# leggedrobotics/delora

Measured on AMD Instinct MI355X. Metric: training scan-pairs/sec, KITTI 64x2048 range images, higher is better.
Workload: dtype f32; 1 GPU; KITTI-shaped 64x2048, batch=8 pairs/GPU, raw scans of ~141k points (ragged, raster order), steps rotate over 8 distinct HBM-resident batches, online normals, ResNet pose CNN (11.9M params, identity-pretrained state), Adam; BASELINE configs[1]; global_batch=8, parallelism=dp1, cnn=fp32, cnn_impl=hip trunk: fp32 MFMA, fused Winograd F(2x2,3x3) + direct implicit GEMM, channels_last=False, hip_graph=False, distinct_batches=8, priming_steps=8

## Files before the change

delora_amd/_lib.py:

```python
import ctypes
import os

_HERE = os.path.dirname(os.path.abspath(__file__))
LIB_PATH = os.path.join(_HERE, "csrc", "libdelora_hip.so")
ABI_VERSION = 10


class DeloraHipError(RuntimeError):
    pass


class SensorStruct(ctypes.Structure):
    _fields_ = [("H", ctypes.c_int32), ("W", ctypes.c_int32),
                ("hfov0", ctypes.c_double), ("hfov1", ctypes.c_double),
                ("vfov0", ctypes.c_double), ("vfov1", ctypes.c_double)]


_vp, _i32, _i64, _u32, _f32, _sz = (ctypes.c_void_p, ctypes.c_int32, ctypes.c_int64, ctypes.c_uint32,
                                    ctypes.c_float, ctypes.c_size_t)
_SP = ctypes.POINTER(SensorStruct)

SIGNATURES = {
    "dl_abi_version": (_i32, []),
    "dl_last_error": (ctypes.c_char_p, []),
# ... 44 lines not shown
    "dl_wino_weights_f32": (_i32, [_vp, _vp, _vp, _i32, _i32, _vp]),
    "dl_wino_weights_batch_f32": (_i32, [_vp, _i32, _vp]),
    "dl_wino_conv3x3_workspace_bytes": (_sz, [_i32, _i32, _i32, _i32, _i32]),
    "dl_wino_conv3x3_nhwc_f32": (_i32, [_vp, _vp, _vp, _vp, _vp, _i32, _i32, _i32, _i32, _i32, _i32, _u32, _vp, _vp]),
    "dl_wino_strided_takes": (_i32, [_i32, _i32, _i32, _i32, _i32, _i32, _i32, _i32]),
    "dl_wino_strided_weights_floats": (_sz, [_i32, _i32, _i32, _i32]),
    "dl_wino_strided_weights_f32": (_i32, [_vp, _vp, _vp, _i32, _i32, _i32, _i32, _vp]),
    "dl_wino_strided_conv3x3_nhwc_f32": (_i32, [_vp, _vp, _vp, _i32, _i32, _i32, _i32, _i32, _i32, _i32, _i32, _u32, _vp]),
    "dl_wino_strided_dgrad3x3_nhwc_f32": (_i32, [_vp, _vp, _vp, _vp, _vp, _i32, _i32, _i32, _i32, _i32, _i32, _i32, _i32, _u32, _vp]),
    "dl_wino_wgrad_workspace_bytes": (_sz, [_i32, _i32, _i32, _i32, _i32]),
    "dl_wino_wgrad3x3_nhwc_f32": (_i32, [_vp, _vp, _vp, _vp, _i32, _i32, _i32, _i32, _i32, _vp]),
    "dl_pool3x3s12_nhwc_fwd": (_i32, [_vp, _i32, _i32, _i32, _i32, _vp, _vp, _vp]),
    "dl_pool3x3s12_nhwc_bwd": (_i32, [_vp, _vp, _vp, _i32, _i32, _i32, _i32, _i32, _vp, _vp]),
    "dl_stem_wgrad_workspace_bytes": (_sz, [_i32, _i32, _i32]),
    "dl_stem_wgrad_f32": (_i32, [_vp, _vp, _vp, _vp, _i32, _i32, _i32, _i32, _vp, _vp, _vp]),
    "dl_quat_to_T_fwd": (_i32, [_vp, _vp, _i32, ctypes.c_float, _vp, _vp]),
    "dl_quat_to_T_bwd": (_i32, [_vp, _vp, _i32, ctypes.c_float, _vp, _vp, _vp]),
    "dl_mean_hw_nhwc_f32": (_i32, [_vp, _i32, _i32, _i32, _vp, _vp]),
    "dl_conv_weights_h": (_i32, [_vp, _vp, _vp, _i32, _i32, _i32, _i32, _vp]),
    "dl_conv_weights_batch_h": (_i32, [_vp, _i32, _i32, _vp]),
    "dl_conv2d_nhwc_h": (_i32, [_vp, _vp, _vp, _vp, _vp, _i32, _i32, _i32, _i32, _i32, _i32, _i32, _i32, _i32, _i32, _i32, _u32, _vp]),
    "dl_conv2d_dgrad_strided_nhwc_h": (_i32, [_vp, _vp, _vp, _vp, _vp, _i32, _i32, _i32, _i32, _i32, _i32, _i32, _i32, _i32, _i32, _i32,
                                              _u32, _vp, _vp]),
    "dl_cast_f32_to_h": (_i32, [_vp, _vp, _i64, _i32, _vp]),
    "dl_heads_fwd": (_i32, [_vp, _vp, _i32, _i32, _i32, _i32, _i32, _vp, _vp, _vp, _vp, _vp, _vp, _vp]),
    "dl_heads_bwd_workspace_bytes": (_sz, [_i32, _i32, _i32, _i32]),
    "dl_heads_bwd": (_i32, [_vp, _vp, _i32, _i32, _i32, _i32, _i32, _vp, _vp, _vp, _vp, _vp, _vp, _vp, _vp, _vp, _vp]),
    "dl_heads_fwd_drop": (_i32, [_vp, _vp, _i32, _i32, _i32, _i32, _i32, _vp, _vp, _vp, _vp, _vp, _vp, _vp, _vp]),
    "dl_heads_bwd_drop": (_i32, [_vp, _vp, _i32, _i32, _i32, _i32, _i32, _vp, _vp, _vp, _vp, _vp, _vp, _vp, _vp, _vp, _vp, _vp]),
    "dl_heads_single_fwd": (_i32, [_vp, _vp, _i32, _i32, _i32, _i32, _i32, _i32, _i32, _i32, _vp, _vp, _vp, _vp, _vp, _vp, _vp]),
# ... 142 lines not shown
```

delora_amd/csrc/common.h:

```cpp
#pragma once
#include <hip/hip_runtime.h>
#include <stdint.h>

#include "../../include/delora_hip.h"

#define DL_WAVE 64
#define DL_BLOCK 256

struct SensorK {
  int H, W, HW;
  float hf0f, hspanf, wm1f;
  float vf0f, vspanf, hm1f;
  double hf0, hres, vf0, vres;
  float tol_u, tol_v;
};

static inline SensorK make_sensor(const dl_sensor* s) {
  SensorK k;
  k.H = s->H; k.W = s->W; k.HW = s->H * s->W;
  k.hf0f = (float)s->hfov0; k.hspanf = (float)(s->hfov1 - s->hfov0); k.wm1f = (float)(s->W - 1);
  k.vf0f = (float)s->vfov0; k.vspanf = (float)(s->vfov1 - s->vfov0); k.hm1f = (float)(s->H - 1);
  k.hf0 = s->hfov0; k.hres = (s->hfov1 - s->hfov0) / (double)(s->W - 1);
  k.vf0 = s->vfov0; k.vres = (s->vfov1 - s->vfov0) / (double)(s->H - 1);
  k.tol_u = (float)(3e-6 * fabs((double)k.wm1f / (double)k.hspanf) + 2.4e-7 * (double)s->W);
// ... 39 lines not shown
  p = __builtin_fmaf(p, t, 0.020650655031204224f);
  p = __builtin_fmaf(p, t, -0.05374353006482124f);
  p = __builtin_fmaf(p, t, 0.13331492245197296f);
  p = __builtin_fmaf(p, t, -0.3333328366279602f);
  const float lo = __builtin_fmaf(ax * t, p, ax);
  const float e = __builtin_amdgcn_exp2f(ax * 2.885390081777927f);
  const float hi = __builtin_fmaf(__builtin_amdgcn_rcpf(e + 1.f), -2.f, 1.f);
  return __builtin_copysignf(ax < 0.625f ? lo : hi, x);
}

extern thread_local char g_dl_err[256];
int dl_fail(int code, const char* fmt, ...);
int dl_check_launch(const char* what);
void dl_plan_batch(const int* tiles, const int* chunks, int n, int machines, int partial_cost, int* nslabs);
int dl_fill_words(void* p, uint32_t value, size_t n_words, hipStream_t st);

#include <hip/hip_ext.h>
struct DlProfTag {
  const char* kernel;
  const char* pass;
  int N, H, W, C, K;
  int ks, sh, sw;
  double flop;
  double bytes;
};
bool dl_prof_is_open();
void dl_prof_events(const DlProfTag& tag, hipEvent_t* e0, hipEvent_t* e1);

struct DlPlanSink {
  char* buf;
// ... 26 lines not shown
```

delora_amd/csrc/infer.hip:

```cpp
#include <stdint.h>
#include <stdio.h>
#include <string.h>

#include "common.h"

typedef uint32_t u32x4i __attribute__((ext_vector_type(4)));

__global__ __launch_bounds__(DL_BLOCK) void k_interleave_pair(const uint32_t* __restrict__ prev, size_t prev_ss, const uint32_t* __restrict__ cur,
                                                              size_t cur_ss, uint32_t HW, uint32_t total, u32x4i* __restrict__ x8) {
  const uint32_t i = blockIdx.x * DL_BLOCK + threadIdx.x;
  if (i >= total) return;
  const uint32_t b = i / HW, p = i - b * HW;
  const uint32_t* a = prev + (size_t)b * prev_ss + p;
  const uint32_t* c = cur + (size_t)b * cur_ss + p;
  const u32x4i lo = {a[0], a[HW], a[2 * (size_t)HW], a[3 * (size_t)HW]};
  const u32x4i hi = {c[0], c[HW], c[2 * (size_t)HW], c[3 * (size_t)HW]};
  x8[2 * (size_t)i] = lo;
  x8[2 * (size_t)i + 1] = hi;
}

__global__ void k_single_scan_offsets(int32_t* __restrict__ offs, int32_t n) {
  if (threadIdx.x < 2) offs[threadIdx.x] = threadIdx.x ? n : 0;
}

namespace {

constexpr size_t kAlign = 256;
inline size_t align_up(size_t n) { return (n + kAlign - 1) / kAlign * kAlign; }
inline int ceil_div(int n, int s) { return (n + s - 1) / s; }

int pose_check(const char* who, const dl_pose_net* net, int B, int H, int W) {
  if (!net) return dl_fail(DL_ERR_INVALID_ARGUMENT, "%s: null net", who);
  if (net->act != DL_POSE_ACT_TANH && net->act != DL_POSE_ACT_RELU)
    return dl_fail(DL_ERR_UNSUPPORTED, "%s: act=%d is not served (1 tanh, 2 relu)", who, net->act);
// ... 90 lines not shown
  if (!rc) return DL_OK;
  char inner[160];
  snprintf(inner, sizeof(inner), "%s", g_dl_err);
  if (block >= 0) return dl_fail(rc, "%s: blocks[%d].%s: %s", who, block, what, inner);
  return dl_fail(rc, "%s: %s: %s", who, what, inner);
}

int pose_forward(const char* who, const dl_pose_net* net, const PosePlan& p, const void* prepared, const float* image_prev, int64_t prev_ss,
                 const float* image_cur, int64_t cur_ss, int B, int H, int W, void* workspace, float* translation, float* quaternion, float* T,
                 dl_stream stream) {
  char* const ws = (char*)workspace;
  float* slot[4];
  for (int i = 0; i < 4; ++i) slot[i] = (float*)(ws + p.slot_off[i]);
  void* const split_ws = p.split_bytes ? (void*)(ws + p.split_off) : nullptr;
  const int act = net->act;
  hipStream_t st = (hipStream_t)stream;
  const uint32_t total = (uint32_t)B * H * W;
  hipLaunchKernelGGL(k_interleave_pair, dim3((total + DL_BLOCK - 1) / DL_BLOCK), dim3(DL_BLOCK), 0, st, (const uint32_t*)image_prev, (size_t)prev_ss,
                     (const uint32_t*)image_cur, (size_t)cur_ss, (uint32_t)(H * W), total, (u32x4i*)slot[0]);
  if (int rc = dl_check_launch(who)) return rc;
  if (int rc = at_layer(who, "conv1", -1, dl_conv2d_nhwc_f32(slot[0], net->conv1_w, slot[1], nullptr, nullptr, B, H, W, 8, 64, 3, 1, 2, 0, act, DL_CONV_ACT, stream)))
    return rc;
  if (int rc = at_layer(who, "pooling", -1, dl_pool3x3s12_nhwc_fwd(slot[1], B, H, W / 2, 64, slot[2], (int8_t*)(ws + p.win_off), stream))) return rc;
  const float* u = (const float*)prepared;
  int s = 2, h = H, w = W / 4;
  for (int i = 0; i < net->n_blocks; ++i) {
    const dl_pose_block& b = net->blocks[i];
    const int ho = ceil_div(h, b.stride_h), wo = ceil_div(w, b.stride_w);
    const float* x = slot[s];
    float *y1 = slot[(s + 1) & 3], *sc = slot[(s + 2) & 3], *y2 = slot[(s + 3) & 3];
    int rc;
    if (runs_wino(b.stride_h, b.stride_w)) {
      rc = dl_wino_conv3x3_nhwc_f32(x, u, y1, nullptr, nullptr, B, h, w, b.cin, b.cout, act, DL_CONV_ACT, split_ws, stream);
      u += dl_wino_weights_floats(b.cout, b.cin);
    } else {
      rc = dl_conv2d_nhwc_f32(x, b.w1, y1, nullptr, nullptr, B, h, w, b.cin, b.cout, 3, b.stride_h, b.stride_w, 0, act, DL_CONV_ACT, stream);
    }
    if ((rc = at_layer(who, "w1", i, rc))) return rc;
// ... 118 lines not shown
```

delora_amd/csrc/stem.hip:

```cpp
#include "common.h"

#define ST_TANH 1
#define ST_RELU 2

typedef float f32x4s __attribute__((ext_vector_type(4)));

__global__ __launch_bounds__(DL_BLOCK) void k_pool_nhwc_fwd(const float* __restrict__ a, int H, int Wc, int C4, uint32_t total,
                                                            float* __restrict__ y, int8_t* __restrict__ win) {
  const uint32_t i = blockIdx.x * DL_BLOCK + threadIdx.x;
  if (i >= total) return;
  const int Wp = Wc >> 1;
  const uint32_t pix = i / (uint32_t)C4;
  const int c4 = (int)(i - pix * (uint32_t)C4);
  const uint32_t nr = pix / (uint32_t)Wp;
  const int q = (int)(pix - nr * (uint32_t)Wp);
  const int r = (int)(nr % (uint32_t)H);
  const int first = r > 0 ? 0 : 3;
  f32x4s best = {-INFINITY, -INFINITY, -INFINITY, -INFINITY};
  int k0 = first, k1 = first, k2 = first, k3 = first;
#pragma unroll
  for (int dh = -1; dh <= 1; ++dh) {
    if (r + dh < 0 || r + dh >= H) continue;
    const float* row = a + ((size_t)(nr + dh) * Wc) * (size_t)(4 * C4) + 4 * c4;
#pragma unroll
    for (int dw = -1; dw <= 1; ++dw) {
      int j = 2 * q + dw;
      j = j < 0 ? j + Wc : j;
      const f32x4s v = *reinterpret_cast<const f32x4s*>(row + (size_t)j * (4 * C4));
      const int k = (dh + 1) * 3 + dw + 1;
      if (v.x > best.x || v.x != v.x) { best.x = v.x; k0 = k; }
      if (v.y > best.y || v.y != v.y) { best.y = v.y; k1 = k; }
      if (v.z > best.z || v.z != v.z) { best.z = v.z; k2 = k; }
      if (v.w > best.w || v.w != v.w) { best.w = v.w; k3 = k; }
    }
  }
  *reinterpret_cast<f32x4s*>(y + (size_t)i * 4) = best;
  *reinterpret_cast<uint32_t*>(win + (size_t)i * 4) = (uint32_t)k0 | ((uint32_t)k1 << 8) | ((uint32_t)k2 << 16) | ((uint32_t)k3 << 24);
}

__device__ __forceinline__ f32x4s pool_bwd_value(const float* __restrict__ g, const float* __restrict__ a, const int8_t* __restrict__ win,
                                                 int H, int Wc, int C4, int act, uint32_t nr, int r, int j, int c4) {
  const int Wp = Wc >> 1;
  const int q0 = j >> 1, col0 = 1 + (j & 1);
  const int q1 = (q0 + 1 == Wp) ? 0 : q0 + 1;
  const bool two = (j & 1) != 0;
  uint32_t w4[6];
  f32x4s gv[6];
  uint32_t code[6];
#pragma unroll
  for (int d = -1; d <= 1; ++d) {
    const bool row_ok = r + d >= 0 && r + d < H;
    const size_t rowbase = (size_t)(nr + (row_ok ? d : 0)) * Wp;
#pragma unroll
    for (int t = 0; t < 2; ++t) {
      const int i = (d + 1) * 2 + t;
      const size_t e = ((rowbase + ((t && two) ? q1 : q0)) * (size_t)C4 + c4) * 4;
      w4[i] = *reinterpret_cast<const uint32_t*>(win + e);
      gv[i] = *reinterpret_cast<const f32x4s*>(g + e);
      code[i] = (row_ok && (t == 0 || two)) ? (uint32_t)((1 - d) * 3 + (t ? 0 : col0)) : 0xffu;
    }
  }
  f32x4s acc = {0.f, 0.f, 0.f, 0.f};
#pragma unroll
  for (int i = 0; i < 6; ++i) {
    acc.x += (w4[i] & 0xffu) == code[i] ? gv[i].x : 0.f;
    acc.y += ((w4[i] >> 8) & 0xffu) == code[i] ? gv[i].y : 0.f;
    acc.z += ((w4[i] >> 16) & 0xffu) == code[i] ? gv[i].z : 0.f;
    acc.w += (w4[i] >> 24) == code[i] ? gv[i].w : 0.f;
  }
  const f32x4s av = *reinterpret_cast<const f32x4s*>(a + (((size_t)nr * Wc + j) * C4 + c4) * 4);
  f32x4s out;
  if (act == ST_TANH) {
    out.x = acc.x * (1.f - av.x * av.x); out.y = acc.y * (1.f - av.y * av.y);
    out.z = acc.z * (1.f - av.z * av.z); out.w = acc.w * (1.f - av.w * av.w);
  } else if (act == ST_RELU) {
    out.x = av.x <= 0.f ? 0.f : acc.x; out.y = av.y <= 0.f ? 0.f : acc.y;
    out.z = av.z <= 0.f ? 0.f : acc.z; out.w = av.w <= 0.f ? 0.f : acc.w;
  } else {
    out = acc;
  }
  return out;
}

__global__ __launch_bounds__(DL_BLOCK) void k_pool_nhwc_bwd(const float* __restrict__ g, const float* __restrict__ a,
                                                            const int8_t* __restrict__ win, int H, int Wc, int C4, int act,
                                                            uint32_t total, float* __restrict__ g_conv) {
  const uint32_t i = blockIdx.x * DL_BLOCK + threadIdx.x;
  if (i >= total) return;
  const uint32_t pix = i / (uint32_t)C4;
  const int c4 = (int)(i - pix * (uint32_t)C4);
  const uint32_t nr = pix / (uint32_t)Wc;
  const int j = (int)(pix - nr * (uint32_t)Wc);
  const int r = (int)(nr % (uint32_t)H);
  *reinterpret_cast<f32x4s*>(g_conv + (size_t)i * 4) = pool_bwd_value(g, a, win, H, Wc, C4, act, nr, r, j, c4);
}

#define SG_PX 64
#define SG_XCOLS (2 * SG_PX + 2)
typedef float f32x16s __attribute__((ext_vector_type(16)));

__global__ __launch_bounds__(DL_BLOCK, 2) void k_stem_wgrad(const float* __restrict__ g, const float* __restrict__ a,
                                                            const int8_t* __restrict__ win, const float* __restrict__ x8, int N, int H,
                                                            int Wc, int act, int chunks_per_slab, float* __restrict__ part) {
  constexpr int K = 64, C4 = 16;
  __shared__ __attribute__((aligned(16))) float gc[SG_PX * K];
  __shared__ __attribute__((aligned(16))) float xt[3 * SG_XCOLS * 8];
  const int tid = threadIdx.x, lane = tid & 63, wave = tid >> 6;
  const int li = lane & 31, half = lane >> 5;
  const int W = 2 * Wc;
  const int cpr = (Wc + SG_PX - 1) / SG_PX;
  const int total = N * H * cpr;
  const int ch_begin = blockIdx.x * chunks_per_slab, ch_end = min(ch_begin + chunks_per_slab, total);
  f32x16s acc[2][3];
#pragma unroll
  for (int i = 0; i < 2; ++i)
#pragma unroll
    for (int j = 0; j < 3; ++j)
#pragma unroll
      for (int r = 0; r < 16; ++r) acc[i][j][r] = 0.f;
  int b_off[3];
#pragma unroll
  for (int ns = 0; ns < 3; ++ns) {
    const int j = min(li + 32 * ns, 71), tap = j >> 3, c = j & 7;
    b_off[ns] = ((tap / 3) * SG_XCOLS + (tap % 3)) * 8 + c;
  }
  for (int ch = ch_begin; ch < ch_end; ++ch) {
    const int cb = ch % cpr;
    const uint32_t nr = (uint32_t)(ch / cpr);
    const int h = (int)(nr % (uint32_t)H), wc0 = cb * SG_PX;
    __syncthreads();
#pragma unroll
    for (int it = 0; it < SG_PX * C4 / DL_BLOCK; ++it) {
      const int q = tid + it * DL_BLOCK, pl = q / C4, c4 = q % C4;
      f32x4s v = {0.f, 0.f, 0.f, 0.f};
      if (wc0 + pl < Wc) v = pool_bwd_value(g, a, win, H, Wc, C4, act, nr, h, wc0 + pl, c4);
      *reinterpret_cast<f32x4s*>(gc + pl * K + c4 * 4) = v;
    }
    for (int q = tid; q < 3 * SG_XCOLS * 2; q += DL_BLOCK) {
      const int hp = q & 1, col = (q >> 1) % SG_XCOLS, row = (q >> 1) / SG_XCOLS;
      const int hh = h + row - 1;
      int w = (2 * wc0 - 1 + col) % W;
      w = w < 0 ? w + W : w;
      f32x4s v = {0.f, 0.f, 0.f, 0.f};
      if (hh >= 0 && hh < H) v = *reinterpret_cast<const f32x4s*>(x8 + (((size_t)(nr + row - 1)) * W + w) * 8 + hp * 4);
      *reinterpret_cast<f32x4s*>(xt + (row * SG_XCOLS + col) * 8 + hp * 4) = v;
    }
    __syncthreads();
#pragma unroll
    for (int ks = 0; ks < 8; ++ks) {
      const int pl = wave * 16 + ks * 2 + half;
      const float a0 = gc[pl * K + li], a1 = gc[pl * K + 32 + li];
      float b[3];
#pragma unroll
      for (int ns = 0; ns < 3; ++ns) b[ns] = xt[b_off[ns] + 2 * pl * 8];
#pragma unroll
      for (int ns = 0; ns < 3; ++ns) {
        acc[0][ns] = __builtin_amdgcn_mfma_f32_32x32x2f32(a0, b[ns], acc[0][ns], 0, 0, 0);
        acc[1][ns] = __builtin_amdgcn_mfma_f32_32x32x2f32(a1, b[ns], acc[1][ns], 0, 0, 0);
      }
    }
// ... 108 lines not shown
  if (N <= 0 || H <= 0 || W <= 0 || W % 4) return 0;
  return (size_t)stem_wgrad_slabs(N * H * ((W / 2 + SG_PX - 1) / SG_PX)) * 64 * 72 * sizeof(float);
}

extern "C" int dl_stem_wgrad_f32(const float* g_pooled, const float* a, const int8_t* win, const float* x8, int32_t N, int32_t H,
                                 int32_t W, int32_t act, void* workspace, float* dw, dl_stream stream) {
  if (!g_pooled || !a || !win || !x8 || !workspace || !dw || N <= 0 || H <= 0 || W <= 0 || act < 0 || act > 2)
    return dl_fail(DL_ERR_INVALID_ARGUMENT, "dl_stem_wgrad_f32: bad argument");
  if (W % 4 || (size_t)N * H * W * 32 >= ((size_t)1 << 32))
    return dl_fail(DL_ERR_UNSUPPORTED, "dl_stem_wgrad_f32: N=%d H=%d W=%d not supported (W %% 4, conv1 output below 2^32 elements)", N, H, W);
  const int Wc = W / 2, total = N * H * ((Wc + SG_PX - 1) / SG_PX), nslabs = stem_wgrad_slabs(total);
  const int cps = (total + nslabs - 1) / nslabs, grid = (total + cps - 1) / cps;
  hipStream_t st = (hipStream_t)stream;
  const DlProfTag tag{"k_stem_wgrad", "wgrad", N, H, W, 8, 64, 3, 1, 2, 2.0 * N * H * Wc * 64.0 * 72.0,
                      4.0 * ((double)N * H * Wc * 64 * 1.5 + (double)N * H * W * 8) + (double)N * H * (Wc / 2) * 64};
  DL_LAUNCH(tag, k_stem_wgrad, dim3(grid), dim3(DL_BLOCK), st, g_pooled, a, win, x8, N, H, Wc, act, cps, (float*)workspace);
  hipLaunchKernelGGL(k_stem_wgrad_reduce, dim3(64 * 72 / 64), dim3(DL_BLOCK), 0, st, (const float*)workspace, grid, dw);
  return dl_check_launch("dl_stem_wgrad_f32");
}
```

delora_amd/models/ring_conv.py:

```python
import ctypes
import os

import torch

from .. import _lib

ACT = {"none": 0, "tanh": 1, "relu": 2}
USE_WINOGRAD = True
EPI_ADD, EPI_ACT, EPI_DACT, EPI_ADD_GRID = 1, 2, 4, 8


def _ptr(t):
    return ctypes.c_void_p(t.data_ptr()) if t is not None else ctypes.c_void_p(0)


def _stream():
    return ctypes.c_void_p(torch.cuda.current_stream().cuda_stream)


ALLOC_SKEW = 0
_skew_state = {"i": 0}


def _empty(shape, dtype, device):
# ... 282 lines not shown
    y = torch.empty((N, H, W // 2, C), dtype=torch.float32, device=a.device)
    win = torch.empty((N, H, W // 2, C), dtype=torch.int8, device=a.device)
    _lib.check(lib.dl_pool3x3s12_nhwc_fwd(_ptr(a), N, H, W, C, _ptr(y), _ptr(win), _stream()), "dl_pool3x3s12_nhwc_fwd")
    return y, win


def pool_bwd(g, a, win, act):
    lib = _lib.load()
    N, H, W, C = a.shape
    out = torch.empty_like(a)
    _lib.check(lib.dl_pool3x3s12_nhwc_bwd(_ptr(g), _ptr(a), _ptr(win), N, H, W, C, int(act), _ptr(out), _stream()),
               "dl_pool3x3s12_nhwc_bwd")
    return out


class MeanHW(torch.autograd.Function):

    @staticmethod
    def forward(ctx, x):
        lib = _lib.load()
        x = x.contiguous()
        N, H, W, C = x.shape
        y = torch.empty((N, C), dtype=torch.float32, device=x.device)
        _lib.check(lib.dl_mean_hw_nhwc_f32(_ptr(x), N, H * W, C, _ptr(y), _stream()), "dl_mean_hw_nhwc_f32")
        ctx.shape = (N, H, W, C)
        return y

    @staticmethod
    def backward(ctx, g):
        N, H, W, C = ctx.shape
# ... 79 lines not shown

def stem_supported(x_shape, out_channels):
    N, C, H, W = x_shape
    k_ok = out_channels % 64 == 0 or (C == 8 and out_channels in NARROW_STEM_CHANNELS and N * H * W * 64 < (1 << 31))
    return ((C % 8 == 0 and C % 16 != 0) or C == TOWER_CHANNELS) and k_ok and W % 4 == 0 and W >= 4 and H >= 1


def planar_stem_supported(x_shape, out_channels):
    return stem_supported(x_shape, out_channels) and x_shape[1] % 16 != 0


class RingStem(torch.autograd.Function):

    @staticmethod
    def forward(ctx, x, w1, act, *drop):
        if drop and drop[0] is not None:
            seed, p = drop[0]
            x8 = stem_input_drop(x, seed, p)
            ctx.drop_p = float(p)
        else:
            seed = None
            x8 = x.permute(0, 2, 3, 1).contiguous()
        ctx.n_extra = len(drop)
        conv1 = conv_nhwc if w1.shape[0] % 64 == 0 else narrow_conv
        a = conv1(x8, weight_storage(w1), stride=(1, 2), act=act, epilogue=EPI_ACT if act else 0)
        y, win = pool_fwd(a)
        ctx.save_for_backward(x8, a, win, w1, *([seed] if seed is not None else []))
        ctx.act = act
        return y

    @staticmethod
    def backward(ctx, g):
        x8, a, win, w1, *seed = ctx.saved_tensors
        extra = (None,) * ctx.n_extra
        want_x = ctx.needs_input_grad[0]
        lib = _lib.load()
        N, H, W, _ = x8.shape
        nbytes = 0 if want_x or a.shape[3] != 64 or x8.shape[3] != 8 else lib.dl_stem_wgrad_workspace_bytes(N, H, W)
        if nbytes:
            ws = torch.empty((nbytes // 4,), dtype=torch.float32, device=x8.device)
            dw = torch.empty((64, 8, 3, 3), dtype=torch.float32, device=x8.device)
            _lib.check(lib.dl_stem_wgrad_f32(_ptr(g.contiguous()), _ptr(a), _ptr(win), _ptr(x8), N, H, W, int(ctx.act), _ptr(ws), _ptr(dw),
                                             _stream()), "dl_stem_wgrad_f32")
            return (None, dw, None) + extra
        gc = pool_bwd(g.contiguous(), a, win, ctx.act)
        if not want_x and a.shape[3] % 64:
            dw = narrow_wgrad(x8, gc, 3, stride=(1, 2)).permute(0, 3, 1, 2)
            return (None, dw if tuple(dw.stride()) == tuple(w1.stride()) else dw.contiguous(), None) + extra
        xp = torch.cat((x8[:, :, -1:], x8, x8[:, :, :1]), dim=2).permute(0, 3, 1, 2)
        gx, dw, _ = torch.ops.aten.convolution_backward(gc.permute(0, 3, 1, 2), xp, w1, None, (1, 2), (1, 0), (1, 1), False,
                                                        (0, 0), 1, (want_x, True, False))
        if want_x:
            gxp = gx
            gx = gxp[..., 1:-1].clone()
            gx[..., -1] += gxp[..., 0]
            gx[..., 0] += gxp[..., -1]
            if seed:
                gx = gx * dropout_scale(seed[0], SITE_INPUT, ctx.drop_p, x8.numel()).view(x8.shape).permute(0, 3, 1, 2)
        return ((gx if want_x else None), dw, None) + extra
# ... 603 lines not shown
```

include/delora_hip.h:

```cpp
#ifndef DELORA_HIP_H
#define DELORA_HIP_H

#include <stddef.h>
#include <stdint.h>

#ifdef __cplusplus
extern "C" {
#endif

#define DL_ABI_VERSION 10

typedef void* dl_stream;

typedef enum {
  DL_OK = 0,
  DL_ERR_INVALID_ARGUMENT = -1,
  DL_ERR_LAUNCH = -2,
  DL_ERR_UNSUPPORTED = -3
} dl_status;

typedef struct {
  int32_t H;
  int32_t W;
  double hfov0, hfov1;
// ... 197 lines not shown
int dl_conv2d_wgrad_nhwc_h(const void* x, const void* g, float* dw, void* workspace, int32_t N, int32_t H, int32_t W, int32_t C,
                           int32_t K, int32_t ksize, int32_t stride_h, int32_t stride_w, int32_t dtype, dl_stream stream);

typedef dl_wgrad_layer dl_wgrad_h_layer;
size_t dl_conv2d_wgrad_batch_h_workspace_bytes(const dl_wgrad_h_layer* layers, int32_t n);
int dl_conv2d_wgrad_batch_nhwc_h(const dl_wgrad_h_layer* layers, int32_t n, void* workspace, int32_t dtype, dl_stream stream);

int dl_pool3x3s12_nhwc_fwd(const float* a, int32_t N, int32_t H, int32_t W, int32_t C, float* y, int8_t* win, dl_stream stream);
int dl_pool3x3s12_nhwc_bwd(const float* g, const float* a, const int8_t* win, int32_t N, int32_t H, int32_t W, int32_t C,
                           int32_t act, float* g_conv, dl_stream stream);

size_t dl_stem_wgrad_workspace_bytes(int32_t N, int32_t H, int32_t W);
int dl_stem_wgrad_f32(const float* g_pooled, const float* a, const int8_t* win, const float* x8, int32_t N, int32_t H, int32_t W,
                      int32_t act, void* workspace, float* dw, dl_stream stream);

typedef struct {
  const float *fc_w, *fc_b;
  const float *r1_w, *r1_b;
  const float *r3_w, *r3_b;
  const float *t1_w, *t1_b;
  const float *t3_w, *t3_b;
} dl_heads_params;
int dl_heads_fwd(const float* x, const dl_heads_params* params, int32_t B, int32_t F, int32_t R, int32_t Hd, int32_t act, float* a1,
                 float* a2, float* rot_raw, float* translation, float* rotation, float* norm, dl_stream stream);
size_t dl_heads_bwd_workspace_bytes(int32_t B, int32_t F, int32_t R, int32_t Hd);
int dl_heads_bwd(const float* x, const dl_heads_params* params, int32_t B, int32_t F, int32_t R, int32_t Hd, int32_t act, const float* a1,
                 const float* a2, const float* rot_raw, const float* norm, const float* grad_translation, const float* grad_rotation,
                 const dl_heads_params* grads, float* grad_x, void* workspace, dl_stream stream);

int dl_heads_fwd_drop(const float* x, const dl_heads_params* params, int32_t B, int32_t F, int32_t R, int32_t Hd, int32_t act,
// ... 90 lines not shown
```

Measured before the change: 696.0 scan-pairs/s.

## Fuse stem conv1, activation and max-pool into one kernel reading NCHW input

Adds a fused stem forward kernel that reads the NCHW (or channels-last dropout) input directly, applies the 3x3 stride-(1,2) conv, the activation and the 3x3 pool, and writes only the pooled output plus window indices. The full-resolution conv1 activation and the NHWC permute copy are never materialised. A matching wgrad path rebuilds the activation value from the pooled output and window index instead of reading the saved conv output. The intent is to cut HBM traffic on the largest activation in the network. When the input gradient is needed, backward recomputes conv1, which adds work in that case.

```diff
diff --git a/delora_amd/_lib.py b/delora_amd/_lib.py
--- a/delora_amd/_lib.py
+++ b/delora_amd/_lib.py
@@ -82,6 +82,9 @@
     "dl_pool3x3s12_nhwc_bwd": (_i32, [_vp, _vp, _vp, _i32, _i32, _i32, _i32, _i32, _vp, _vp]),
     "dl_stem_wgrad_workspace_bytes": (_sz, [_i32, _i32, _i32]),
     "dl_stem_wgrad_f32": (_i32, [_vp, _vp, _vp, _vp, _i32, _i32, _i32, _i32, _vp, _vp, _vp]),
+    "dl_stem_fwd_f32": (_i32, [_vp, _i64, _i64, _i64, _i64, _vp, _i32, _i32, _i32, _i32, _vp, _vp, _vp]),
+    "dl_stem_fwd_plan": (_i32, [_i32, _i32, _vp, _vp, _vp, _vp]),
+    "dl_stem_wgrad_y_f32": (_i32, [_vp, _vp, _vp, _vp, _i64, _i64, _i64, _i64, _i32, _i32, _i32, _i32, _vp, _vp, _vp]),
     "dl_quat_to_T_fwd": (_i32, [_vp, _vp, _i32, ctypes.c_float, _vp, _vp]),
     "dl_quat_to_T_bwd": (_i32, [_vp, _vp, _i32, ctypes.c_float, _vp, _vp, _vp]),
     "dl_mean_hw_nhwc_f32": (_i32, [_vp, _i32, _i32, _i32, _vp, _vp]),
diff --git a/delora_amd/csrc/common.h b/delora_amd/csrc/common.h
--- a/delora_amd/csrc/common.h
+++ b/delora_amd/csrc/common.h
@@ -77,6 +77,8 @@
 int dl_check_launch(const char* what);
 void dl_plan_batch(const int* tiles, const int* chunks, int n, int machines, int partial_cost, int* nslabs);
 int dl_fill_words(void* p, uint32_t value, size_t n_words, hipStream_t st);
+int dl_stem_fwd_launch(const char* who, const float* x_lo, int64_t sn_lo, const float* x_hi, int64_t sn_hi, int64_t sc, int64_t sh, int64_t sp,
+                       const float* w, int32_t N, int32_t H, int32_t W, int32_t act, float* y, int8_t* win, dl_stream stream);
 
 #include <hip/hip_ext.h>
 struct DlProfTag {
diff --git a/delora_amd/csrc/infer.hip b/delora_amd/csrc/infer.hip
--- a/delora_amd/csrc/infer.hip
+++ b/delora_amd/csrc/infer.hip
@@ -3,21 +3,6 @@
 #include <string.h>
 
 #include "common.h"
-
-typedef uint32_t u32x4i __attribute__((ext_vector_type(4)));
-
-__global__ __launch_bounds__(DL_BLOCK) void k_interleave_pair(const uint32_t* __restrict__ prev, size_t prev_ss, const uint32_t* __restrict__ cur,
-                                                              size_t cur_ss, uint32_t HW, uint32_t total, u32x4i* __restrict__ x8) {
-  const uint32_t i = blockIdx.x * DL_BLOCK + threadIdx.x;
-  if (i >= total) return;
-  const uint32_t b = i / HW, p = i - b * HW;
-  const uint32_t* a = prev + (size_t)b * prev_ss + p;
-  const uint32_t* c = cur + (size_t)b * cur_ss + p;
-  const u32x4i lo = {a[0], a[HW], a[2 * (size_t)HW], a[3 * (size_t)HW]};
-  const u32x4i hi = {c[0], c[HW], c[2 * (size_t)HW], c[3 * (size_t)HW]};
-  x8[2 * (size_t)i] = lo;
-  x8[2 * (size_t)i + 1] = hi;
-}
 
 __global__ void k_single_scan_offsets(int32_t* __restrict__ offs, int32_t n) {
   if (threadIdx.x < 2) offs[threadIdx.x] = threadIdx.x ? n : 0;
@@ -138,14 +123,9 @@
   for (int i = 0; i < 4; ++i) slot[i] = (float*)(ws + p.slot_off[i]);
   void* const split_ws = p.split_bytes ? (void*)(ws + p.split_off) : nullptr;
   const int act = net->act;
-  hipStream_t st = (hipStream_t)stream;
-  const uint32_t total = (uint32_t)B * H * W;
-  hipLaunchKernelGGL(k_interleave_pair, dim3((total + DL_BLOCK - 1) / DL_BLOCK), dim3(DL_BLOCK), 0, st, (const uint32_t*)image_prev, (size_t)prev_ss,
-                     (const uint32_t*)image_cur, (size_t)cur_ss, (uint32_t)(H * W), total, (u32x4i*)slot[0]);
-  if (int rc = dl_check_launch(who)) return rc;
-  if (int rc = at_layer(who, "conv1", -1, dl_conv2d_nhwc_f32(slot[0], net->conv1_w, slot[1], nullptr, nullptr, B, H, W, 8, 64, 3, 1, 2, 0, act, DL_CONV_ACT, stream)))
+  if (int rc = at_layer(who, "stem", -1, dl_stem_fwd_launch("dl_stem_fwd_f32", image_prev, prev_ss, image_cur, cur_ss, (int64_t)H * W, W, 1, net->conv1_w,
+                                                            B, H, W, act, slot[2], (int8_t*)(ws + p.win_off), stream)))
     return rc;
-  if (int rc = at_layer(who, "pooling", -1, dl_pool3x3s12_nhwc_fwd(slot[1], B, H, W / 2, 64, slot[2], (int8_t*)(ws + p.win_off), stream))) return rc;
   const float* u = (const float*)prepared;
   int s = 2, h = H, w = W / 4;
   for (int i = 0; i < net->n_blocks; ++i) {
diff --git a/delora_amd/csrc/stem.hip b/delora_amd/csrc/stem.hip
--- a/delora_amd/csrc/stem.hip
+++ b/delora_amd/csrc/stem.hip
@@ -38,6 +38,7 @@
   *reinterpret_cast<uint32_t*>(win + (size_t)i * 4) = (uint32_t)k0 | ((uint32_t)k1 << 8) | ((uint32_t)k2 << 16) | ((uint32_t)k3 << 24);
 }
 
+template <bool FROM_Y>
 __device__ __forceinline__ f32x4s pool_bwd_value(const float* __restrict__ g, const float* __restrict__ a, const int8_t* __restrict__ win,
                                                  int H, int Wc, int C4, int act, uint32_t nr, int r, int j, int c4) {
   const int Wp = Wc >> 1;
@@ -47,6 +48,7 @@
   uint32_t w4[6];
   f32x4s gv[6];
   uint32_t code[6];
+  uint32_t eo[6];
 #pragma unroll
   for (int d = -1; d <= 1; ++d) {
     const bool row_ok = r + d >= 0 && r + d < H;
@@ -57,18 +59,35 @@
       const size_t e = ((rowbase + ((t && two) ? q1 : q0)) * (size_t)C4 + c4) * 4;
       w4[i] = *reinterpret_cast<const uint32_t*>(win + e);
       gv[i] = *reinterpret_cast<const f32x4s*>(g + e);
+      eo[i] = (uint32_t)e;
       code[i] = (row_ok && (t == 0 || two)) ? (uint32_t)((1 - d) * 3 + (t ? 0 : col0)) : 0xffu;
     }
   }
   f32x4s acc = {0.f, 0.f, 0.f, 0.f};
+  constexpr uint32_t NONE = 0xffffffffu;
+  uint32_t ex = NONE, ey = NONE, ez = NONE, ew = NONE;
 #pragma unroll
   for (int i = 0; i < 6; ++i) {
-    acc.x += (w4[i] & 0xffu) == code[i] ? gv[i].x : 0.f;
-    acc.y += ((w4[i] >> 8) & 0xffu) == code[i] ? gv[i].y : 0.f;
-    acc.z += ((w4[i] >> 16) & 0xffu) == code[i] ? gv[i].z : 0.f;
-    acc.w += (w4[i] >> 24) == code[i] ? gv[i].w : 0.f;
-  }
-  const f32x4s av = *reinterpret_cast<const f32x4s*>(a + (((size_t)nr * Wc + j) * C4 + c4) * 4);
+    const bool mx = (w4[i] & 0xffu) == code[i], my = ((w4[i] >> 8) & 0xffu) == code[i];
+    const bool mz = ((w4[i] >> 16) & 0xffu) == code[i], mw = (w4[i] >> 24) == code[i];
+    acc.x += mx ? gv[i].x : 0.f;
+    acc.y += my ? gv[i].y : 0.f;
+    acc.z += mz ? gv[i].z : 0.f;
+    acc.w += mw ? gv[i].w : 0.f;
+    if (FROM_Y) {
+      ex = mx ? eo[i] : ex; ey = my ? eo[i] : ey;
+      ez = mz ? eo[i] : ez; ew = mw ? eo[i] : ew;
+    }
+  }
+  f32x4s av;
+  if (FROM_Y && act == 0) {
+    av = (f32x4s){0.f, 0.f, 0.f, 0.f};
+  } else if (FROM_Y) {
+    av.x = ex != NONE ? a[ex] : 0.f; av.y = ey != NONE ? a[ey + 1] : 0.f;
+    av.z = ez != NONE ? a[ez + 2] : 0.f; av.w = ew != NONE ? a[ew + 3] : 0.f;
+  } else {
+    av = *reinterpret_cast<const f32x4s*>(a + (((size_t)nr * Wc + j) * C4 + c4) * 4);
+  }
   f32x4s out;
   if (act == ST_TANH) {
     out.x = acc.x * (1.f - av.x * av.x); out.y = acc.y * (1.f - av.y * av.y);
@@ -92,19 +111,23 @@
   const uint32_t nr = pix / (uint32_t)Wc;
   const int j = (int)(pix - nr * (uint32_t)Wc);
   const int r = (int)(nr % (uint32_t)H);
-  *reinterpret_cast<f32x4s*>(g_conv + (size_t)i * 4) = pool_bwd_value(g, a, win, H, Wc, C4, act, nr, r, j, c4);
+  *reinterpret_cast<f32x4s*>(g_conv + (size_t)i * 4) = pool_bwd_value<false>(g, a, win, H, Wc, C4, act, nr, r, j, c4);
 }
 
 #define SG_PX 64
 #define SG_XCOLS (2 * SG_PX + 2)
+#define SG_XPAD 3
+#define SG_XALLOC (SG_XCOLS + 2 * SG_XPAD)
 typedef float f32x16s __attribute__((ext_vector_type(16)));
 
+struct StemStrides { long n, c, h, p; };
+template <bool FROM_Y>
 __global__ __launch_bounds__(DL_BLOCK, 2) void k_stem_wgrad(const float* __restrict__ g, const float* __restrict__ a,
-                                                            const int8_t* __restrict__ win, const float* __restrict__ x8, int N, int H,
-                                                            int Wc, int act, int chunks_per_slab, float* __restrict__ part) {
+                                                            const int8_t* __restrict__ win, const float* __restrict__ x8, StemStrides xs,
+                                                            int N, int H, int Wc, int act, int chunks_per_slab, float* __restrict__ part) {
   constexpr int K = 64, C4 = 16;
   __shared__ __attribute__((aligned(16))) float gc[SG_PX * K];
-  __shared__ __attribute__((aligned(16))) float xt[3 * SG_XCOLS * 8];
+  __shared__ __attribute__((aligned(16))) float xt[3 * SG_XALLOC * 8];
   const int tid = threadIdx.x, lane = tid & 63, wave = tid >> 6;
   const int li = lane & 31, half = lane >> 5;
   const int W = 2 * Wc;
@@ -122,28 +145,73 @@
 #pragma unroll
   for (int ns = 0; ns < 3; ++ns) {
     const int j = min(li + 32 * ns, 71), tap = j >> 3, c = j & 7;
-    b_off[ns] = ((tap / 3) * SG_XCOLS + (tap % 3)) * 8 + c;
+    b_off[ns] = ((tap / 3) * SG_XALLOC + SG_XPAD + (tap % 3)) * 8 + c;
   }
   for (int ch = ch_begin; ch < ch_end; ++ch) {
     const int cb = ch % cpr;
     const uint32_t nr = (uint32_t)(ch / cpr);
     const int h = (int)(nr % (uint32_t)H), wc0 = cb * SG_PX;
+    const int wb = wc0 > 0 ? 2 * wc0 - 1 : W - 1;
     __syncthreads();
 #pragma unroll
     for (int it = 0; it < SG_PX * C4 / DL_BLOCK; ++it) {
       const int q = tid + it * DL_BLOCK, pl = q / C4, c4 = q % C4;
       f32x4s v = {0.f, 0.f, 0.f, 0.f};
-      if (wc0 + pl < Wc) v = pool_bwd_value(g, a, win, H, Wc, C4, act, nr, h, wc0 + pl, c4);
+      if (wc0 + pl < Wc) v = pool_bwd_value<FROM_Y>(g, a, win, H, Wc, C4, act, nr, h, wc0 + pl, c4);
       *reinterpret_cast<f32x4s*>(gc + pl * K + c4 * 4) = v;
     }
+    const bool dense_cl = !FROM_Y || (xs.c == 1 && xs.p == 8 && xs.h == 8L * W && xs.n == xs.h * H);
+    if (FROM_Y && !dense_cl && xs.p == 1 && !((xs.n | xs.c | xs.h) & 3) && !((uintptr_t)x8 & 15)) {
+      const float* xi = x8 + (long)(nr / (uint32_t)H) * xs.n;
+      constexpr int NG = (SG_XALLOC + 3) / 4, NX = 3 * 8 * NG, NX_IT = (NX + DL_BLOCK - 1) / DL_BLOCK;
+      const int wg0 = wc0 > 0 ? 2 * wc0 - 4 : W - 4;
+      f32x4s xv[NX_IT];
+#pragma unroll
+      for (int it = 0; it < NX_IT; ++it) {
+        const int q = min(tid + it * DL_BLOCK, NX - 1);
+        const int c = q & 7, gi = (q >> 3) % NG, row = (q >> 3) / NG;
+        const int hh = h + row - 1;
+        int w = wg0 + 4 * gi;
+        if (w >= W) { w -= W; if (w >= W) w %= W; }
+        const f32x4s v = *reinterpret_cast<const f32x4s*>(xi + c * xs.c + min(max(hh, 0), H - 1) * xs.h + w);
+        xv[it] = (hh >= 0 && hh < H) ? v : (f32x4s){0.f, 0.f, 0.f, 0.f};
+      }
+#pragma unroll
+      for (int it = 0; it < NX_IT; ++it) {
+        const int q = min(tid + it * DL_BLOCK, NX - 1);
+        const int c = q & 7, gi = (q >> 3) % NG, row = (q >> 3) / NG;
+        float* d = xt + (row * SG_XALLOC + 4 * gi) * 8 + c;
+        d[0] = xv[it].x; d[8] = xv[it].y; d[16] = xv[it].z; d[24] = xv[it].w;
+      }
+    } else if (FROM_Y && !dense_cl) {
+      const float* xi = x8 + (long)(nr / (uint32_t)H) * xs.n;
+      constexpr int NX = 3 * SG_XCOLS * 8, NX_IT = (NX + DL_BLOCK - 1) / DL_BLOCK;
+      float xv[NX_IT];
+#pragma unroll
+      for (int it = 0; it < NX_IT; ++it) {
+        const int q = min(tid + it * DL_BLOCK, NX - 1);
+        const int col = q % SG_XCOLS, t2 = q / SG_XCOLS, c = t2 & 7, row = t2 >> 3;
+        const int hh = h + row - 1;
+        int w = wb + col;
+        if (w >= W) { w -= W; if (w >= W) w %= W; }
+        const float v = xi[c * xs.c + min(max(hh, 0), H - 1) * xs.h + w * xs.p];
+        xv[it] = (hh >= 0 && hh < H) ? v : 0.f;
+      }
+#pragma unroll
+      for (int it = 0; it < NX_IT; ++it) {
+        const int q = min(tid + it * DL_BLOCK, NX - 1);
+        const int col = q % SG_XCOLS, t2 = q / SG_XCOLS, c = t2 & 7, row = t2 >> 3;
+        xt[(row * SG_XALLOC + SG_XPAD + col) * 8 + c] = xv[it];
+      }
+    } else
     for (int q = tid; q < 3 * SG_XCOLS * 2; q += DL_BLOCK) {
       const int hp = q & 1, col = (q >> 1) % SG_XCOLS, row = (q >> 1) / SG_XCOLS;
       const int hh = h + row - 1;
-      int w = (2 * wc0 - 1 + col) % W;
-      w = w < 0 ? w + W : w;
+      int w = wb + col;
+      if (w >= W) { w -= W; if (w >= W) w %= W; }
       f32x4s v = {0.f, 0.f, 0.f, 0.f};
       if (hh >= 0 && hh < H) v = *reinterpret_cast<const f32x4s*>(x8 + (((size_t)(nr + row - 1)) * W + w) * 8 + hp * 4);
-      *reinterpret_cast<f32x4s*>(xt + (row * SG_XCOLS + col) * 8 + hp * 4) = v;
+      *reinterpret_cast<f32x4s*>(xt + (row * SG_XALLOC + SG_XPAD + col) * 8 + hp * 4) = v;
     }
     __syncthreads();
 #pragma unroll
@@ -282,7 +350,206 @@
   hipStream_t st = (hipStream_t)stream;
   const DlProfTag tag{"k_stem_wgrad", "wgrad", N, H, W, 8, 64, 3, 1, 2, 2.0 * N * H * Wc * 64.0 * 72.0,
                       4.0 * ((double)N * H * Wc * 64 * 1.5 + (double)N * H * W * 8) + (double)N * H * (Wc / 2) * 64};
-  DL_LAUNCH(tag, k_stem_wgrad, dim3(grid), dim3(DL_BLOCK), st, g_pooled, a, win, x8, N, H, Wc, act, cps, (float*)workspace);
+  DL_LAUNCH(tag, k_stem_wgrad<false>, dim3(grid), dim3(DL_BLOCK), st, g_pooled, a, win, x8, StemStrides{0, 0, 0, 0}, N, H, Wc, act, cps,
+            (float*)workspace);
   hipLaunchKernelGGL(k_stem_wgrad_reduce, dim3(64 * 72 / 64), dim3(DL_BLOCK), 0, st, (const float*)workspace, grid, dw);
   return dl_check_launch("dl_stem_wgrad_f32");
 }
+
+extern "C" int dl_stem_wgrad_y_f32(const float* g_pooled, const float* y, const int8_t* win, const float* x, int64_t stride_n,
+                                   int64_t stride_c, int64_t stride_h, int64_t stride_w, int32_t N, int32_t H, int32_t W, int32_t act,
+                                   void* workspace, float* dw, dl_stream stream) {
+  if (!g_pooled || !y || !win || !x || !workspace || !dw || N <= 0 || H <= 0 || W <= 0 || act < 0 || act > 2)
+    return dl_fail(DL_ERR_INVALID_ARGUMENT, "dl_stem_wgrad_y_f32: bad argument");
+  if (W % 4 || (size_t)N * H * W * 32 >= ((size_t)1 << 32))
+    return dl_fail(DL_ERR_UNSUPPORTED, "dl_stem_wgrad_y_f32: N=%d H=%d W=%d not supported (W %% 4, conv1 output below 2^32 elements)", N, H, W);
+  if (stride_n < 0 || stride_c < 0 || stride_h < 0 || stride_w < 0)
+    return dl_fail(DL_ERR_INVALID_ARGUMENT, "dl_stem_wgrad_y_f32: negative stride");
+  if (stride_c == 1 && stride_w == 8 && stride_h == 8L * W && stride_n == stride_h * H && ((uintptr_t)x & 15))
+    return dl_fail(DL_ERR_INVALID_ARGUMENT, "dl_stem_wgrad_y_f32: a dense channels-last input must be 16-byte aligned");
+  const int Wc = W / 2, total = N * H * ((Wc + SG_PX - 1) / SG_PX), nslabs = stem_wgrad_slabs(total);
+  const int cps = (total + nslabs - 1) / nslabs, grid = (total + cps - 1) / cps;
+  hipStream_t st = (hipStream_t)stream;
+  const DlProfTag tag{"k_stem_wgrad", "wgrad", N, H, W, 8, 64, 3, 1, 2, 2.0 * N * H * Wc * 64.0 * 72.0,
+                      4.0 * ((double)N * H * Wc * 64 + (double)N * H * W * 8) + (double)N * H * (Wc / 2) * 64};
+  DL_LAUNCH(tag, k_stem_wgrad<true>, dim3(grid), dim3(DL_BLOCK), st, g_pooled, y, win, x,
+            StemStrides{(long)stride_n, (long)stride_c, (long)stride_h, (long)stride_w}, N, H, Wc, act, cps, (float*)workspace);
+  hipLaunchKernelGGL(k_stem_wgrad_reduce, dim3(64 * 72 / 64), dim3(DL_BLOCK), 0, st, (const float*)workspace, grid, dw);
+  return dl_check_launch("dl_stem_wgrad_y_f32");
+}
+
+#define STF_Q 31
+#define STF_R 22
+#define STF_CC (2 * STF_Q + 2)
+#define STF_XC (4 * STF_Q + 3)
+#define STF_XCOLS (2 * STF_CC + 2)
+#define STF_XS 12
+#define STF_AS 68
+#define STF_ITEMS ((STF_XC * 8 + DL_BLOCK - 1) / DL_BLOCK)
+static_assert(STF_CC == 64 && STF_Q * 16 <= 2 * DL_BLOCK, "two pixel subtiles per row; two pooling items per thread");
+
+struct StemFwdArgs {
+  const float* x_lo;
+  const float* x_hi;
+  long sn_lo, sn_hi, sc, sh, sp;
+  const float* w;
+  float* y;
+  int8_t* win;
+  int N, H, W, act, R, bands, tiles;
+};
+
+__device__ __forceinline__ float st_act(float v, int act) {
+  if (act == ST_TANH) return dl_tanh(v);
+  if (act == ST_RELU) return v < 0.f ? 0.f : v;
+  return v;
+}
+
+__global__ __launch_bounds__(DL_BLOCK, 2) void k_stem_fwd(StemFwdArgs a) {
+  __shared__ __attribute__((aligned(16))) float xin[3 * STF_XCOLS * STF_XS];
+  __shared__ __attribute__((aligned(16))) float ring[3 * STF_CC * STF_AS];
+  const int tid = threadIdx.x, lane = tid & 63, wave = tid >> 6;
+  const int li = lane & 31, half = lane >> 5;
+  const int mi = wave >> 1, ni = wave & 1;
+  const int H = a.H, W = a.W, Wp = W >> 2;
+  int b = blockIdx.x;
+  const int tile = b % a.tiles; b /= a.tiles;
+  const int band = b % a.bands, n = b / a.bands;
+  const int r0 = band * a.R, r1 = min(r0 + a.R, H);
+  const int q0 = tile * STF_Q;
+
+  f32x4s wf[9];
+#pragma unroll
+  for (int tap = 0; tap < 9; ++tap) wf[tap] = *reinterpret_cast<const f32x4s*>(a.w + ((ni * 32 + li) * 9 + tap) * 8 + half * 4);
+
+  const float* xp[STF_ITEMS];
+  int xl[STF_ITEMS];
+#pragma unroll
+  for (int it = 0; it < STF_ITEMS; ++it) {
+    const int q = min(tid + it * DL_BLOCK, STF_XC * 8 - 1);
+    const int col = a.sc == 1 ? q >> 3 : q % STF_XC, c = a.sc == 1 ? q & 7 : q / STF_XC;
+    int w = (4 * q0 - 3 + col) % W;
+    w = w < 0 ? w + W : w;
+    xp[it] = (c < 4 ? a.x_lo + n * a.sn_lo + c * a.sc : a.x_hi + n * a.sn_hi + (c - 4) * a.sc) + w * a.sp;
+    xl[it] = col * STF_XS + c;
+  }
+  float xr[STF_ITEMS];
+#define STF_LOAD(HH)                                                                              \
+  {                                                                                               \
+    const bool in_ = (HH) >= 0 && (HH) < H;            \
+    const long ro_ = (long)min(max((HH), 0), H - 1) * a.sh;                                       \
+    _Pragma("unroll") for (int it = 0; it < STF_ITEMS; ++it) xr[it] = xp[it][ro_];                \
+    _Pragma("unroll") for (int it = 0; it < STF_ITEMS; ++it) xr[it] = in_ ? xr[it] : 0.f;         \
+  }
+#define STF_STORE(HH)                                                                             \
+  {                                                                                               \
+    float* s_ = xin + (((HH) + 3) % 3) * (STF_XCOLS * STF_XS);                                    \
+    _Pragma("unroll") for (int it = 0; it < STF_ITEMS; ++it) s_[xl[it]] = xr[it];                 \
+  }
+  if (tid < 3 * (STF_XCOLS - STF_XC) * STF_XS) {
+    const int per = (STF_XCOLS - STF_XC) * STF_XS;
+    xin[(tid / per) * (STF_XCOLS * STF_XS) + STF_XC * STF_XS + tid % per] = 0.f;
+  }
+  const int h_first = max(r0 - 1, 0), h_last = min(r1, H - 1);
+#pragma unroll
+  for (int d = -1; d <= 1; ++d) {
+    STF_LOAD(h_first + d)
+    STF_STORE(h_first + d)
+  }
+  __syncthreads();
+  const int a_off = (2 * (mi * 32 + li)) * STF_XS + half * 4;
+  for (int h = h_first; h <= r1; ++h) {
+    const bool fetch = h + 1 <= h_last;
+    if (fetch) STF_LOAD(h + 2)
+    if (h <= h_last) {
+      f32x16s acc;
+#pragma unroll
+      for (int r = 0; r < 16; ++r) acc[r] = 0.f;
+#pragma unroll
+      for (int tap = 0; tap < 9; ++tap) {
+        const int slot = (h + tap / 3 + 2) % 3;
+        const f32x4s av = *reinterpret_cast<const f32x4s*>(xin + slot * (STF_XCOLS * STF_XS) + a_off + (tap % 3) * STF_XS);
+#pragma unroll
+        for (int j = 0; j < 4; ++j) acc = __builtin_amdgcn_mfma_f32_32x32x2f32(av[j], wf[tap][j], acc, 0, 0, 0);
+      }
+      if (a.act == ST_TANH) {
+#pragma unroll
+        for (int r = 0; r < 16; ++r) acc[r] = st_act(acc[r], ST_TANH);
+      } else if (a.act == ST_RELU) {
+#pragma unroll
+        for (int r = 0; r < 16; ++r) acc[r] = st_act(acc[r], ST_RELU);
+      }
+      float* rs = ring + (h % 3) * (STF_CC * STF_AS) + ni * 32 + li;
+#pragma unroll
+      for (int r = 0; r < 16; ++r) rs[(mi * 32 + (r & 3) + 8 * (r >> 2) + 4 * half) * STF_AS] = acc[r];
+    }
+    __syncthreads();
+    if (fetch) STF_STORE(h + 2)
+    const int r = h - 1;
+    if (r >= r0) {
+      const int first = r > 0 ? 0 : 3;
+      for (int q = tid; q < STF_Q * 16; q += DL_BLOCK) {
+        const int ql = q >> 4, c4 = q & 15;
+        if (q0 + ql >= Wp) continue;
+        f32x4s best = {-INFINITY, -INFINITY, -INFINITY, -INFINITY};
+        int k0 = first, k1 = first, k2 = first, k3 = first;
+#pragma unroll
+        for (int dh = -1; dh <= 1; ++dh) {
+          if (r + dh < 0 || r + dh >= H) continue;
+          const float* row = ring + ((r + dh) % 3) * (STF_CC * STF_AS) + (2 * ql) * STF_AS + 4 * c4;
+#pragma unroll
+          for (int dw = 0; dw < 3; ++dw) {
+            const f32x4s v = *reinterpret_cast<const f32x4s*>(row + dw * STF_AS);
+            const int k = (dh + 1) * 3 + dw;
+            if (v.x > best.x || v.x != v.x) { best.x = v.x; k0 = k; }
+            if (v.y > best.y || v.y != v.y) { best.y = v.y; k1 = k; }
+            if (v.z > best.z || v.z != v.z) { best.z = v.z; k2 = k; }
+            if (v.w > best.w || v.w != v.w) { best.w = v.w; k3 = k; }
+          }
+        }
+        const size_t o = ((((size_t)n * H + r) * Wp + q0 + ql) * 16 + c4) * 4;
+        *reinterpret_cast<f32x4s*>(a.y + o) = best;
+        *reinterpret_cast<uint32_t*>(a.win + o) = (uint32_t)k0 | ((uint32_t)k1 << 8) | ((uint32_t)k2 << 16) | ((uint32_t)k3 << 24);
+      }
+    }
+    __syncthreads();
+  }
+}
+#undef STF_LOAD
+#undef STF_STORE
+
+static void stem_fwd_plan(int H, int W, int* R, int* bands, int* tiles) {
+  *R = STF_R;
+  *bands = (H + STF_R - 1) / STF_R;
+  *tiles = (W / 4 + STF_Q - 1) / STF_Q;
+}
+
+extern "C" int dl_stem_fwd_plan(int32_t H, int32_t W, int32_t* R, int32_t* Q, int32_t* bands, int32_t* tiles) {
+  if (!R || !Q || !bands || !tiles || H <= 0 || W <= 0) return dl_fail(DL_ERR_INVALID_ARGUMENT, "dl_stem_fwd_plan: bad argument");
+  if (W % 4) return dl_fail(DL_ERR_UNSUPPORTED, "dl_stem_fwd_plan: W=%d not supported (W %% 4)", W);
+  int r, b, t;
+  stem_fwd_plan(H, W, &r, &b, &t);
+  *R = r; *Q = STF_Q; *bands = b; *tiles = t;
+  return DL_OK;
+}
+
+int dl_stem_fwd_launch(const char* who, const float* x_lo, int64_t sn_lo, const float* x_hi, int64_t sn_hi, int64_t sc, int64_t sh, int64_t sp,
+                       const float* w, int32_t N, int32_t H, int32_t W, int32_t act, float* y, int8_t* win, dl_stream stream) {
+  if (!x_lo || !x_hi || !w || !y || !win || N <= 0 || H <= 0 || W <= 0 || act < 0 || act > 2 || sn_lo < 0 || sn_hi < 0 || sc < 0 || sh < 0 || sp < 0)
+    return dl_fail(DL_ERR_INVALID_ARGUMENT, "%s: bad argument", who);
+  if ((uintptr_t)w & 15) return dl_fail(DL_ERR_INVALID_ARGUMENT, "%s: the weights are not 16-byte aligned", who);
+  if (W % 4 || (size_t)N * H * W * 32 >= ((size_t)1 << 32))
+    return dl_fail(DL_ERR_UNSUPPORTED, "%s: N=%d H=%d W=%d not supported (W %% 4, conv1 output below 2^32 elements)", who, N, H, W);
+  StemFwdArgs a{x_lo, x_hi, (long)sn_lo, (long)sn_hi, (long)sc, (long)sh, (long)sp, w, y, win, N, H, W, act, 0, 0, 0};
+  stem_fwd_plan(H, W, &a.R, &a.bands, &a.tiles);
+  const double px = (double)N * H * (W / 2);
+  const DlProfTag tag{"k_stem_fwd", "fwd", N, H, W, 8, 64, 3, 1, 2, 2.0 * px * 64.0 * 72.0,
+                      4.0 * ((double)N * H * W * 8 + px * 32 + 64.0 * 72.0) + px * 32};
+  DL_LAUNCH(tag, k_stem_fwd, dim3(N * a.bands * a.tiles), dim3(DL_BLOCK), (hipStream_t)stream, a);
+  return dl_check_launch(who);
+}
+
+extern "C" int dl_stem_fwd_f32(const float* x, int64_t stride_n, int64_t stride_c, int64_t stride_h, int64_t stride_w, const float* w,
+                               int32_t N, int32_t H, int32_t W, int32_t act, float* y, int8_t* win, dl_stream stream) {
+  return dl_stem_fwd_launch("dl_stem_fwd_f32", x, stride_n, x ? x + 4 * stride_c : nullptr, stride_n, stride_c, stride_h, stride_w, w, N, H, W,
+                            act, y, win, stream);
+}
diff --git a/delora_amd/models/ring_conv.py b/delora_amd/models/ring_conv.py
--- a/delora_amd/models/ring_conv.py
+++ b/delora_amd/models/ring_conv.py
@@ -320,6 +320,39 @@
     return out
 
 
+def _stem_strides(x, channels_last):
+    if channels_last:
+        N, H, W, C = x.shape
+        strides = (H * W * C, 1, W * C, C)
+    else:
+        N, C, H, W = x.shape
+        strides = (C * H * W, H * W, W, 1)
+    assert C == 8 and x.is_contiguous() and x.dtype == torch.float32
+    return N, H, W, strides
+
+
+def stem_fwd(x, w_krsc, act, channels_last=False):
+    lib = _lib.load()
+    N, H, W, strides = _stem_strides(x, channels_last)
+    y = torch.empty((N, H, W // 4, 64), dtype=torch.float32, device=x.device)
+    win = torch.empty((N, H, W // 4, 64), dtype=torch.int8, device=x.device)
+    _lib.check(lib.dl_stem_fwd_f32(_ptr(x), *strides, _ptr(w_krsc), N, H, W, int(act), _ptr(y), _ptr(win), _stream()), "dl_stem_fwd_f32")
+    return y, win
+
+
+def stem_wgrad_y(g, y, win, x, act, channels_last=False):
+    lib = _lib.load()
+    N, H, W, strides = _stem_strides(x, channels_last)
+    nbytes = lib.dl_stem_wgrad_workspace_bytes(N, H, W)
+    if not nbytes:
+        raise _lib.DeloraHipError("dl_stem_wgrad_y_f32: N=%d H=%d W=%d not supported" % (N, H, W))
+    ws = torch.empty((nbytes // 4,), dtype=torch.float32, device=x.device)
+    dw = torch.empty((64, 8, 3, 3), dtype=torch.float32, device=x.device)
+    _lib.check(lib.dl_stem_wgrad_y_f32(_ptr(g), _ptr(y), _ptr(win), _ptr(x), *strides, N, H, W, int(act), _ptr(ws), _ptr(dw), _stream()),
+               "dl_stem_wgrad_y_f32")
+    return dw
+
+
 class MeanHW(torch.autograd.Function):
 
     @staticmethod
@@ -429,19 +462,24 @@
 
     @staticmethod
     def forward(ctx, x, w1, act, *drop):
-        if drop and drop[0] is not None:
+        dropped = bool(drop) and drop[0] is not None
+        ctx.n_extra = len(drop)
+        ctx.act = act
+        ctx.fused = w1.shape[0] == 64 and x.shape[1] == 8
+        if dropped:
             seed, p = drop[0]
-            x8 = stem_input_drop(x, seed, p)
             ctx.drop_p = float(p)
-        else:
-            seed = None
-            x8 = x.permute(0, 2, 3, 1).contiguous()
-        ctx.n_extra = len(drop)
+        if ctx.fused:
+            xin = stem_input_drop(x, seed, p) if dropped else x.contiguous()
+            ctx.channels_last = dropped
+            y, win = stem_fwd(xin, weight_storage(w1), act, channels_last=dropped)
+            ctx.save_for_backward(xin, y, win, w1, *([seed] if dropped else []))
+            return y
+        x8 = stem_input_drop(x, seed, p) if dropped else x.permute(0, 2, 3, 1).contiguous()
         conv1 = conv_nhwc if w1.shape[0] % 64 == 0 else narrow_conv
         a = conv1(x8, weight_storage(w1), stride=(1, 2), act=act, epilogue=EPI_ACT if act else 0)
         y, win = pool_fwd(a)
-        ctx.save_for_backward(x8, a, win, w1, *([seed] if seed is not None else []))
-        ctx.act = act
+        ctx.save_for_backward(x8, a, win, w1, *([seed] if dropped else []))
         return y
 
     @staticmethod
@@ -449,15 +487,13 @@
         x8, a, win, w1, *seed = ctx.saved_tensors
         extra = (None,) * ctx.n_extra
         want_x = ctx.needs_input_grad[0]
-        lib = _lib.load()
+        if ctx.fused:
+            xin, y = x8, a
+            if not want_x:
+                return (None, stem_wgrad_y(g.contiguous(), y, win, xin, ctx.act, channels_last=ctx.channels_last), None) + extra
+            x8 = xin if ctx.channels_last else xin.permute(0, 2, 3, 1).contiguous()
+            a = conv_nhwc(x8, weight_storage(w1), stride=(1, 2), act=ctx.act, epilogue=EPI_ACT if ctx.act else 0)
         N, H, W, _ = x8.shape
-        nbytes = 0 if want_x or a.shape[3] != 64 or x8.shape[3] != 8 else lib.dl_stem_wgrad_workspace_bytes(N, H, W)
-        if nbytes:
-            ws = torch.empty((nbytes // 4,), dtype=torch.float32, device=x8.device)
-            dw = torch.empty((64, 8, 3, 3), dtype=torch.float32, device=x8.device)
-            _lib.check(lib.dl_stem_wgrad_f32(_ptr(g.contiguous()), _ptr(a), _ptr(win), _ptr(x8), N, H, W, int(ctx.act), _ptr(ws), _ptr(dw),
-                                             _stream()), "dl_stem_wgrad_f32")
-            return (None, dw, None) + extra
         gc = pool_bwd(g.contiguous(), a, win, ctx.act)
         if not want_x and a.shape[3] % 64:
             dw = narrow_wgrad(x8, gc, 3, stride=(1, 2)).permute(0, 3, 1, 2)
diff --git a/include/delora_hip.h b/include/delora_hip.h
--- a/include/delora_hip.h
+++ b/include/delora_hip.h
@@ -235,6 +235,13 @@
 int dl_stem_wgrad_f32(const float* g_pooled, const float* a, const int8_t* win, const float* x8, int32_t N, int32_t H, int32_t W,
                       int32_t act, void* workspace, float* dw, dl_stream stream);
 
+int dl_stem_fwd_f32(const float* x, int64_t stride_n, int64_t stride_c, int64_t stride_h, int64_t stride_w, const float* w, int32_t N,
+                    int32_t H, int32_t W, int32_t act, float* y, int8_t* win, dl_stream stream);
+int dl_stem_fwd_plan(int32_t H, int32_t W, int32_t* R, int32_t* Q, int32_t* bands, int32_t* tiles);
+int dl_stem_wgrad_y_f32(const float* g_pooled, const float* y, const int8_t* win, const float* x, int64_t stride_n, int64_t stride_c,
+                        int64_t stride_h, int64_t stride_w, int32_t N, int32_t H, int32_t W, int32_t act, void* workspace, float* dw,
+                        dl_stream stream);
+
 typedef struct {
   const float *fc_w, *fc_b;
   const float *r1_w, *r1_b;
```

New measurement: 695.2 scan-pairs/s. No clear change (-0.1%).
